# dmosopt/dmosopt

Measured on NVIDIA H100. Metric: candidate-evals/sec (GP+sort+HV) pop=65536 dim=30 obj=3, higher is better.
Workload: dtype f64 results; GP variance contraction in split-fp16 wgmma with fp32 accumulation (precision=auto: calibrated against the float64 path, 0 of 65535 rows of the last step recomputed in float64); ranks on u32 ids

## Files before the change

dmosopt_b200/csrc/common.cuh:

```cuda
#pragma once

#include <cuda_runtime.h>
#include <math.h>
#include <stdint.h>
#include <stdio.h>

#include <string>
#include <vector>

#include "../../include/dmosopt_b200.h"

struct dmo_ctx {
  int device = 0;
  cudaStream_t stream = nullptr;
  cudaMemPool_t pool = nullptr;
  cudaEvent_t ev0 = nullptr, ev1 = nullptr;
  int sm_count = 132;
  int64_t launches = 0;
  int64_t waits = 0;
  std::string err;
  void* flush_buf = nullptr;
  size_t flush_bytes = 0;
  int* dev_flag = nullptr;
  uint64_t h2d_bytes = 0, d2h_bytes = 0;
// ... 216 lines not shown

__device__ __forceinline__ double warp_sum(double v) {
#pragma unroll
  for (int o = 16; o > 0; o >>= 1) v += __shfl_xor_sync(0xffffffffu, v, o);
  return v;
}

template <int NW>
__device__ __forceinline__ double block_sum(double v, double* red) {
  v = warp_sum(v);
  __syncthreads();
  if ((threadIdx.x & 31) == 0) red[threadIdx.x >> 5] = v;
  __syncthreads();
  double s = 0.0;
#pragma unroll 8
  for (int w = 0; w < NW; ++w) s += red[w];
  __syncthreads();
  return s;
}

#endif

int prim_sort_pairs_u64(dmo_ctx* ctx, const uint64_t* kin, uint64_t* kout, const uint32_t* vin,
                        uint32_t* vout, int64_t n, int begin_bit, int end_bit);
int prim_sort_pairs_u32(dmo_ctx* ctx, const uint32_t* kin, uint32_t* kout, const uint32_t* vin,
                        uint32_t* vout, int64_t n, int begin_bit, int end_bit);
int prim_inclusive_sum_u32(dmo_ctx* ctx, const uint32_t* in, uint32_t* out, int64_t n);
int prim_exclusive_sum_i32(dmo_ctx* ctx, const int32_t* in, int32_t* out, int64_t n);
int prim_inclusive_min_f64(dmo_ctx* ctx, const double* in, double* out, int64_t n);
int prim_iota_u32(dmo_ctx* ctx, uint32_t* out, int64_t n);
int prim_gather_u32(dmo_ctx* ctx, const uint32_t* src, const uint32_t* idx, int64_t n, uint32_t* out);
int prim_round_f32(dmo_ctx* ctx, double* a, int64_t n);
int prim_col_keys(dmo_ctx* ctx, const double* dF, int64_t n, int M, int j, uint64_t* keys, uint32_t* idx);
int prim_sort_by_column(dmo_ctx* ctx, const double* dF, int64_t n, int M, int j, DevBuf<uint32_t>& sidx);

int rank_nd_device(dmo_ctx* ctx, const double* dY, int64_t n, int M, int32_t* d_rank);
int rank_nd_device_keep(dmo_ctx* ctx, const double* dY, int64_t n, int M, int64_t keep, int32_t* d_rank);
int nondominated_flags_device(dmo_ctx* ctx, const double* dY, int64_t n, int M, int32_t* d_flag01);
int nondominated_keep_flags(dmo_ctx* ctx, const double* dF, int64_t n, int M, DevBuf<int32_t>& flag);
int dense_ids(dmo_ctx* ctx, const double* dY, int64_t n, int M, DevBuf<uint32_t>& R, DevBuf<uint32_t>& maxid);
int lex_order(dmo_ctx* ctx, const uint32_t* R, int64_t n, int M, int sshift, DevBuf<uint32_t>& permA, DevBuf<uint32_t>& permB,
              const uint32_t** perm);
int crowding_device(dmo_ctx* ctx, const double* dY, int64_t n, int M, double* dD);
int euclidean_device(dmo_ctx* ctx, const double* dY, int64_t n, int M, double* dD);
int lexsort_device(dmo_ctx* ctx, const int32_t* d_rank, const double* const* d_desc_keys, int nkeys,
                   int64_t n, uint32_t* d_perm, bool rank_below_n);
int hypervolume_device(dmo_ctx* ctx, const double* dF, int64_t n, int M, const double* h_ref, double* h_out);
int hypervolume_device_ranked(dmo_ctx* ctx, const double* dF, int64_t n, int M, const double* h_ref, const int32_t* d_rank,
                              double* h_out);
struct Hv3Ranked {
  int64_t n = 0;
  double ref[3] = {0.0, 0.0, 0.0};
  bool tree = false;
  DevBuf<int32_t> pos;
  DevBuf<double> xs, ys, zs, res;
  DevBuf<uint32_t> zo;
};
int hv3_ranked_enqueue(dmo_ctx* ctx, const double* dF, int64_t n, const double* h_ref, const int32_t* d_rank, Hv3Ranked& s);
int hv3_ranked_finish(dmo_ctx* ctx, Hv3Ranked& s, double* h_out);
int tournament_device(dmo_ctx* ctx, const int32_t* d_rank, const double* d_crowd, int64_t pop, int64_t poolsize, uint64_t seed,
                      uint64_t stream_id, int64_t* d_pool, double* d_u);
int nsga2_generate_device(dmo_ctx* ctx, const double* d_pop_x, int d, const int64_t* d_pool, int64_t poolsize, int64_t popsize,
                          double crossover_prob, double mutation_prob, double mutation_rate, const double* d_dic,
                          const double* d_dim, const double* d_xlb, const double* d_xub, uint64_t seed, uint64_t stream_id,
                          double* d_x_gen, int32_t* d_kind, int64_t* n_children, double* d_draws);
int remove_worst_device(dmo_ctx* ctx, const double* dX, const double* dY, int64_t n, int d, int M, int metric,
                        const double* const* d_extra, int n_extra, int64_t keep, double* dX_out, double* dY_out, int32_t* d_rank_out,
                        int64_t* d_perm_out);
int gather_rows_device(dmo_ctx* ctx, const double* src, const double* alt, const uint8_t* sel, const int64_t* idx, int64_t n,
                       int64_t row_elems, double* dst);
int cmaes_generate_device(dmo_ctx* ctx, const double* parents_x, const double* sigmas, int sigma_cols, const double* A,
                          const int64_t* p_idx, const double* z, int64_t n, int d, const double* xlb, const double* xub, double* x_out);
int cmaes_step_z_device(dmo_ctx* ctx, const double* x_gen, const int64_t* cand_idx, const double* parents_x, const int64_t* par_idx,
                        const double* xlb, const double* xub, const double* steps, int64_t n, int d, double* z_out);
int scale_rows_device(dmo_ctx* ctx, double* rows, int64_t row_elems, int64_t n_seg, const int64_t* seg_row, const int64_t* seg_start,
                      const double* factors);
int cmaes_update_cholesky_device(dmo_ctx* ctx, double* A, double* Ainv, double* pc, const double* z, const double* psucc, int64_t n, int d,
                                 double cc, double ccov, double pthresh);
int ehvi_select_device(dmo_ctx* ctx, const double* F, int64_t nf, const double* means, const double* variances, int64_t nc, int M,
                       const double* ref, int nds, int64_t k, int64_t* sel, double* score);
int feas_rank_device(dmo_ctx* ctx, const dmo_feas* m, const double* dX, int64_t n, double* d_rank);
int feas_model_dim(const dmo_feas* m);
```

dmosopt_b200/csrc/gp.cuh:

```cuda
#pragma once
#include <vector>

#include "common.cuh"

struct GpVarOps {
  int64_t Npad = 0;
  int G = 0;
  std::vector<double> h_kscale;
  DevBuf<double> Linv;
  bool tensor_ready = false;
  DevBuf<uint16_t> Lhi, Llo;
  DevBuf<float> Lscale;
  DevBuf<int> Kexp;
  int alloc(dmo_ctx* ctx, int64_t N, int G);
};

struct dmo_gp {
  int64_t N = 0;
  int d = 0, M = 0, kernel = 0;
  bool isotropic = true;
  GpVarOps ops;
  std::vector<int> h_cov, h_lead;
  DevBuf<int> cov;
  DevBuf<double> Xt;
// ... 15 lines not shown
  double cal_mean_err_only = 0.0;
  double cal_var_err = 0.0;
  double refine_theta = 1.0;
  int64_t last_refined = 0;
};

__device__ __forceinline__ double stationary(double s2, int kind) {
  if (kind == DMO_KERNEL_MATERN52) {
    const double K = sqrt(s2) * 2.23606797749978969641;
    return (1.0 + K + K * K / 3.0) * exp(-K);
  }
  return exp(-0.5 * s2);
}

constexpr int64_t GP_MAX_CHUNK = (int64_t)1 << 20;

int gp_predict_fp64(dmo_ctx* ctx, dmo_gp* gp, const double* dXn, int64_t P, double* d_mean, double* d_var);

int gp_linv_from_factor(dmo_ctx* ctx, const double* L, int64_t N, int64_t ldo, double* dst);
int gp_linv_from_factor_batched(dmo_ctx* ctx, const double* L, int64_t ldl, int64_t sL, int64_t N, int nbat, int64_t ldo,
                                int64_t sdst, double* dst);
int gp_fit_batched(dmo_ctx* ctx, int64_t N, int d, int nbat, int kernel, const double* X, const double* inv_ls, const double* constant,
                   const double* diag_add, const double* y, double* A, int64_t ld, int* info, double* work, double* alpha, double* lml);
int gp_potrf_batched(dmo_ctx* ctx, double* A, int64_t ld, int nbat, int* info);
constexpr int GP_F64_TILE = 128;
int gp_var_contract_fp64(dmo_ctx* ctx, const GpVarOps& ops, const double* Ks, int64_t kplane, int64_t Pcpad, int nsplit,
                         double* vnorm, int64_t vn_ld);
int gp_prepare_tensor(dmo_ctx* ctx, GpVarOps& ops);
constexpr int GP_TC_TILE = 128;
int gp_tensor_var_planes(int64_t Npad);
int gp_var_contract_tensor(dmo_ctx* ctx, const GpVarOps& ops, const uint16_t* Kh, const uint16_t* Kl, int64_t k_alloc,
                           int64_t k_rows, int64_t Pcpad, double* vnorm, int64_t vn_ld, int* abort_flag, int free_sms = 0);
#ifndef DMO_GP_LANE_SMS
#define DMO_GP_LANE_SMS 14
#endif
constexpr int GP_LANE_SMS = DMO_GP_LANE_SMS;
struct GpOverlap {
  cudaEvent_t mean_ready = nullptr;
};
int gp_predict_tensor(dmo_ctx* ctx, dmo_gp* gp, const double* dXn, int64_t P, double* d_mean, double* d_var,
                      int* abort_flag = nullptr, const GpOverlap* ov = nullptr, bool var_route_mean = false);
extern const char* const GP_WATCHDOG_MSG;
struct GpPending {
  GpOverlap ov;
  bool active = false;
  int64_t P = 0;
  const double* dXn = nullptr;
  double *d_mean = nullptr, *d_var = nullptr;
  DevBuf<double> xn;
  DevBuf<int32_t> flag, pos;
};
int gp_predict_device(dmo_ctx* ctx, dmo_gp* gp, const double* dX, int64_t P, double* d_mean, double* d_var, int precision,
                      GpPending* pending = nullptr, bool var_route_mean = false);
int gp_predict_finish(dmo_ctx* ctx, dmo_gp* gp, GpPending& pending, bool* refined);

struct GpUnitPredict {
  const char* who = "";
  bool tensor = false;
  int64_t tile = 0;
  int64_t Pc_alloc = 0;
  int n_vp = 0;
  DevBuf<double> vnorm, Ks;
  DevBuf<uint16_t> Kh, Kl;
  DevBuf<int> abort_flag;
  int check(dmo_ctx* ctx, const char* who, int precision, int d);
  int alloc(dmo_ctx* ctx, int64_t P, int64_t Npad, int planes, bool want_var);
  int contract(dmo_ctx* ctx, const GpVarOps& ops, int64_t Pcpad);
// ... 67 lines not shown
```

dmosopt_b200/csrc/hv.cu:

```cuda
#include <stdlib.h>
#include <string.h>

#include "common.cuh"

int hv_many_device(dmo_ctx* ctx, const double* Fnd, const uint32_t* sidx, int64_t n, int M, const double* dref, double* h_out);
int hv3_tree_device(dmo_ctx* ctx, const double* xs, const double* ys, const double* zs, const uint32_t* zo, int64_t n, double rx,
                    double ry, double rz, double* partial, int64_t* n_partial);

namespace {

constexpr int HV_T = 128;

__global__ void inside_flag_kernel(const double* __restrict__ F, int64_t n, int M, const double* __restrict__ ref,
                                   const int32_t* __restrict__ drop, int32_t* __restrict__ flag) {
  int64_t i = (int64_t)blockIdx.x * blockDim.x + threadIdx.x;
  if (i > n) return;
  if (i == n) {
    flag[i] = 0;
    return;
  }
  bool in = drop == nullptr || drop[i] == 0;
  for (int j = 0; j < M; ++j) in = in && (ref[j] > F[i * M + j]);
  flag[i] = in ? 1 : 0;
}
// ... 556 lines not shown
    DMO_TRY(sum_partials(ctx, part_main, n2 * tiles, &t_main));
    DMO_TRY(sum_partials(ctx, part_a, nbv, &t_a));
    if (M == 5) DMO_TRY(sum_partials(ctx, part_b, nbv, &t_b));
    *h_out = (M == 4) ? (t_a - t_main) : (t_a - t_b + t_main);
    return DMO_OK;
  }
  DevBuf<uint32_t> sz, zinv, zo;
  DevBuf<double> xs, ys, zs;
  DMO_TRY(prim_sort_by_column(ctx, Fnd.p, n2, M, 2, sz));
  DMO_TRY(zinv.alloc(ctx, n2));
  DMO_TRY(zo.alloc(ctx, n2));
  DMO_TRY(xs.alloc(ctx, n2));
  DMO_TRY(ys.alloc(ctx, n2));
  DMO_TRY(zs.alloc(ctx, n2));
  const unsigned g = (unsigned)ceil_div(n2, 256);
  DMO_LAUNCH(invert_perm_kernel, g, 256, 0, sz.p, n2, zinv.p);
  DMO_TRY(prim_gather_u32(ctx, zinv.p, sx.p, n2, zo.p));
  DMO_LAUNCH(gather_col_kernel, g, 256, 0, Fnd.p, sx.p, n2, M, 0, xs.p);
  DMO_LAUNCH(gather_col_kernel, g, 256, 0, Fnd.p, sx.p, n2, M, 1, ys.p);
  DMO_LAUNCH(gather_col_kernel, g, 256, 0, Fnd.p, sx.p, n2, M, 2, zs.p);
  int64_t nb = ceil_div(n2, HV_T);
  DevBuf<double> partial;
  DMO_TRY(partial.alloc(ctx, nb));
  if (n2 >= hv3_tree_min()) {
    DMO_TRY(hv3_tree_device(ctx, xs.p, ys.p, zs.p, zo.p, n2, h_ref[0], h_ref[1], h_ref[2], partial.p, &nb));
  } else {
    ProfileScope ps(ctx, "hv3");
    DMO_LAUNCH(hv3_kernel, (unsigned)nb, HV_T, 0, xs.p, ys.p, zs.p, zo.p, n2, h_ref[0], h_ref[1], h_ref[2], partial.p);
  }
  DMO_TRY(sum_partials(ctx, partial, nb, h_out));
  return DMO_OK;
}

int hv3_ranked_enqueue(dmo_ctx* ctx, const double* dF, int64_t n, const double* h_ref, const int32_t* d_rank, Hv3Ranked& s) {
  s.n = n;
  memcpy(s.ref, h_ref, sizeof(s.ref));
  s.tree = n >= hv3_tree_min();
  DevBuf<double> dref, Fin;
  DevBuf<int32_t> flag;
  DevBuf<uint32_t> sx, sz, zinv;
  DMO_TRY(dref.alloc(ctx, 3));
  DMO_CUDA(cudaMemcpyAsync(dref.p, h_ref, 3 * sizeof(double), cudaMemcpyHostToDevice, ctx->stream));
  DMO_TRY(flag.alloc(ctx, n + 1));
  DMO_TRY(s.pos.alloc(ctx, n + 1));
  DMO_TRY(Fin.alloc(ctx, (size_t)n * 3));
  const unsigned g = (unsigned)ceil_div(n, 256);
  DMO_LAUNCH(inside_flag_kernel, (unsigned)ceil_div(n + 1, 256), 256, 0, dF, n, 3, dref.p, d_rank, flag.p);
  DMO_TRY(prim_exclusive_sum_i32(ctx, flag.p, s.pos.p, n + 1));
  DMO_LAUNCH(compact_rows_kernel, g, 256, 0, dF, n, 3, flag.p, s.pos.p, Fin.p);
  DMO_LAUNCH(pad_rows_kernel, g, 256, 0, Fin.p, n, 3, s.pos.p + n, dref.p);
  DMO_TRY(prim_sort_by_column(ctx, Fin.p, n, 3, 0, sx));
  DMO_TRY(prim_sort_by_column(ctx, Fin.p, n, 3, 2, sz));
  DMO_TRY(zinv.alloc(ctx, n));
  DMO_TRY(s.zo.alloc(ctx, n));
  DMO_TRY(s.xs.alloc(ctx, n));
  DMO_TRY(s.ys.alloc(ctx, n));
  DMO_TRY(s.zs.alloc(ctx, n));
  DMO_LAUNCH(invert_perm_kernel, g, 256, 0, sz.p, n, zinv.p);
  DMO_TRY(prim_gather_u32(ctx, zinv.p, sx.p, n, s.zo.p));
  DMO_LAUNCH(gather_col_kernel, g, 256, 0, Fin.p, sx.p, n, 3, 0, s.xs.p);
  DMO_LAUNCH(gather_col_kernel, g, 256, 0, Fin.p, sx.p, n, 3, 1, s.ys.p);
  DMO_LAUNCH(gather_col_kernel, g, 256, 0, Fin.p, sx.p, n, 3, 2, s.zs.p);
  if (s.tree) {
    DevBuf<double> partial;
    int64_t nb = ceil_div(n, HV_T);
    DMO_TRY(partial.alloc(ctx, nb));
    DMO_TRY(hv3_tree_device(ctx, s.xs.p, s.ys.p, s.zs.p, s.zo.p, n, h_ref[0], h_ref[1], h_ref[2], partial.p, &nb));
    DMO_TRY(s.res.alloc(ctx, 1));
    DMO_LAUNCH(final_sum_kernel, 1, 256, 0, partial.p, nb, s.res.p);
  }
  DMO_CHECK_LAUNCH();
  return DMO_OK;
}

int hv3_ranked_finish(dmo_ctx* ctx, Hv3Ranked& s, double* h_out) {
  *h_out = 0.0;
  int32_t n1 = 0;
  DMO_CUDA(cudaMemcpyAsync(&n1, s.pos.p + s.n, sizeof(int32_t), cudaMemcpyDeviceToHost, ctx->stream));
  DMO_CUDA(dmo_wait(ctx));
  if (n1 == 0) return DMO_OK;
  if (s.tree && n1 >= hv3_tree_min()) {
    DMO_CUDA(cudaMemcpyAsync(h_out, s.res.p, sizeof(double), cudaMemcpyDeviceToHost, ctx->stream));
    DMO_CUDA(dmo_wait(ctx));
    return DMO_OK;
  }
// ... 140 lines not shown
```

dmosopt_b200/csrc/prims.cu:

```cuda
#include <cub/cub.cuh>

#include "common.cuh"

int prim_sort_pairs_u64(dmo_ctx* ctx, const uint64_t* kin, uint64_t* kout, const uint32_t* vin,
                        uint32_t* vout, int64_t n, int begin_bit, int end_bit) {
  if (n <= 0) return DMO_OK;
  size_t tmp = 0;
  DMO_CUDA(cub::DeviceRadixSort::SortPairs(nullptr, tmp, kin, kout, vin, vout, (int)n, begin_bit, end_bit,
                                           ctx->stream));
  DevBuf<uint8_t> t;
  DMO_TRY(t.alloc(ctx, tmp));
  DMO_CUDA(cub::DeviceRadixSort::SortPairs(t.p, tmp, kin, kout, vin, vout, (int)n, begin_bit, end_bit,
                                           ctx->stream));
  ctx->launches += 1 + (end_bit - begin_bit + 7) / 8;
  return DMO_OK;
}

int prim_sort_pairs_u32(dmo_ctx* ctx, const uint32_t* kin, uint32_t* kout, const uint32_t* vin,
                        uint32_t* vout, int64_t n, int begin_bit, int end_bit) {
  if (n <= 0) return DMO_OK;
  size_t tmp = 0;
  DMO_CUDA(cub::DeviceRadixSort::SortPairs(nullptr, tmp, kin, kout, vin, vout, (int)n, begin_bit, end_bit,
                                           ctx->stream));
  DevBuf<uint8_t> t;
// ... 62 lines not shown
int prim_gather_u32(dmo_ctx* ctx, const uint32_t* src, const uint32_t* idx, int64_t n, uint32_t* out) {
  if (n <= 0) return DMO_OK;
  DMO_LAUNCH(gather_u32_kernel, (unsigned)ceil_div(n, 256), 256, 0, src, idx, n, out);
  DMO_CHECK_LAUNCH();
  return DMO_OK;
}

__global__ void round_f32_kernel(double* a, int64_t n) {
  int64_t i = (int64_t)blockIdx.x * blockDim.x + threadIdx.x;
  if (i < n) a[i] = (double)(float)a[i];
}

int prim_round_f32(dmo_ctx* ctx, double* a, int64_t n) {
  if (n <= 0) return DMO_OK;
  DMO_LAUNCH(round_f32_kernel, (unsigned)ceil_div(n, 256), 256, 0, a, n);
  DMO_CHECK_LAUNCH();
  return DMO_OK;
}

__global__ void col_key_kernel(const double* __restrict__ F, int64_t n, int M, int j, uint64_t* __restrict__ keys,
                               uint32_t* __restrict__ idx) {
  int64_t i = (int64_t)blockIdx.x * blockDim.x + threadIdx.x;
  if (i < n) {
    keys[i] = f64_to_ordered(F[i * M + j]);
    idx[i] = (uint32_t)i;
  }
}

int prim_col_keys(dmo_ctx* ctx, const double* dF, int64_t n, int M, int j, uint64_t* keys, uint32_t* idx) {
  DMO_LAUNCH(col_key_kernel, (unsigned)ceil_div(n, 256), 256, 0, dF, n, M, j, keys, idx);
  return DMO_OK;
}

int prim_sort_by_column(dmo_ctx* ctx, const double* dF, int64_t n, int M, int j, DevBuf<uint32_t>& sidx) {
  DevBuf<uint64_t> k0, k1;
  DevBuf<uint32_t> i0;
  DMO_TRY(k0.alloc(ctx, n));
  DMO_TRY(k1.alloc(ctx, n));
  DMO_TRY(i0.alloc(ctx, n));
  DMO_TRY(sidx.alloc(ctx, n));
  DMO_TRY(prim_col_keys(ctx, dF, n, M, j, k0.p, i0.p));
  return prim_sort_pairs_u64(ctx, k0.p, k1.p, i0.p, sidx.p, n, 0, 64);
}
```

dmosopt_b200/csrc/rank.cu:

```cuda
#include <stdlib.h>

#include <type_traits>

#include "common.cuh"

namespace {

constexpr int RANK_T = 128;

__device__ __forceinline__ int ld_acquire_gpu(const int* p) {
  int v;
  asm volatile("ld.acquire.gpu.global.s32 %0, [%1];" : "=r"(v) : "l"(p) : "memory");
  return v;
}
__device__ __forceinline__ void st_release_gpu(int* p, int v) {
  asm volatile("st.release.gpu.global.s32 [%0], %1;" ::"l"(p), "r"(v) : "memory");
}

__global__ void flag_new_u64_kernel(const uint64_t* __restrict__ skeys, int64_t n, uint32_t* __restrict__ flag) {
  int64_t p = (int64_t)blockIdx.x * blockDim.x + threadIdx.x;
  if (p < n) flag[p] = (p > 0 && skeys[p] != skeys[p - 1]) ? 1u : 0u;
}

__global__ void scatter_dense_kernel(const uint32_t* __restrict__ dense, const uint32_t* __restrict__ sidx, int64_t n,
// ... 706 lines not shown
  const int j2 = M == 3 ? 2 : 1;
  return GridIds{R, R + n, R + (size_t)j2 * n, maxid + 1, maxid + j2};
}

struct CellGrid {
  int gbits = 0;
  DevBuf<uint32_t> cstartA, cstartB;
  DevBuf<uint4> crecA, crecB;
  DevBuf<uint32_t> pm;
  DevBuf<uint32_t> first, slotA, slotB;
};

__global__ void grid_key_kernel(GridIds ids, int64_t n, int gbits, uint32_t* __restrict__ key0, uint32_t* __restrict__ keyA,
                                uint32_t* __restrict__ keyB) {
  const int64_t i = (int64_t)blockIdx.x * blockDim.x + threadIdx.x;
  if (i >= n) return;
  const uint32_t G1 = (1u << gbits) - 1u;
  const uint32_t a = min(ids.c1[i] >> cell_shift(*ids.max1, gbits), G1), b = min(ids.c2[i] >> cell_shift(*ids.max2, gbits), G1);
  key0[i] = ids.c0[i];
  keyA[i] = (a << gbits) | b;
  keyB[i] = (b << gbits) | a;
}

__global__ void grid_gather_kernel(GridIds ids, const uint32_t* __restrict__ order, int64_t n, uint4* __restrict__ crec,
                                   uint32_t* __restrict__ slot) {
  const int64_t t = (int64_t)blockIdx.x * blockDim.x + threadIdx.x;
  if (t >= n) return;
  const uint32_t i = order[t];
  crec[t] = make_uint4(ids.c0[i], ids.c1[i], ids.c2[i], i);
  if (slot != nullptr) slot[i] = (uint32_t)t;
}

__global__ void grid_start_kernel(const uint32_t* __restrict__ skey, int64_t n, int ncell, uint32_t* __restrict__ cstart) {
  int c = blockIdx.x * blockDim.x + threadIdx.x;
  if (c > ncell) return;
  int64_t lo = 0, hi = n;
  while (lo < hi) {
    const int64_t mid = (lo + hi) >> 1;
    if (skey[mid] < (uint32_t)c) lo = mid + 1; else hi = mid;
  }
  cstart[c] = (uint32_t)lo;
}

__global__ void grid_cellmin_kernel(const uint32_t* __restrict__ cstart, const uint4* __restrict__ crec, int ncell,
                                    uint32_t* __restrict__ first, uint32_t* __restrict__ pm) {
  const int c = blockIdx.x * blockDim.x + threadIdx.x;
  if (c >= ncell) return;
  uint32_t f = first != nullptr ? first[c] : cstart[c];
  const uint32_t e = cstart[c + 1];
  while (f < e && crec[f].x == PEEL_DEAD) ++f;
  if (first != nullptr) first[c] = f;
  pm[c] = f < e ? crec[f].x : PEEL_DEAD;
}

__global__ void grid_prefix_min_kernel(uint32_t* __restrict__ pm, int gbits, int pass) {
  extern __shared__ uint32_t sh_scan[];
  const int G = 1 << gbits;
  const int line = blockIdx.x, t = threadIdx.x;
  const int cell = pass == 0 ? line * G + t : t * G + line;
  uint32_t v = pm[cell];
  sh_scan[t] = v;
  __syncthreads();
  for (int off = 1; off < G; off <<= 1) {
    const uint32_t o = t >= off ? sh_scan[t - off] : PEEL_DEAD;
    __syncthreads();
    v = min(v, o);
    sh_scan[t] = v;
    __syncthreads();
  }
  pm[cell] = v;
}

template <typename OutT>
__global__ void grid_flag_kernel(GridIds ids, int64_t n, int gbits, const uint32_t* __restrict__ pm,
                                 const uint32_t* __restrict__ cstartA, const uint32_t* __restrict__ cstartB,
                                 const uint4* __restrict__ crecA, const uint4* __restrict__ crecB,
                                 const uint8_t* __restrict__ alive, OutT* __restrict__ dom_out) {
  const int64_t i = (int64_t)blockIdx.x * blockDim.x + threadIdx.x;
  if (i >= n || (alive != nullptr && !alive[i])) return;
  const int G = 1 << gbits;
  const uint32_t c0 = ids.c0[i], c1 = ids.c1[i], c2 = ids.c2[i];
  const int a = (int)min(c1 >> cell_shift(*ids.max1, gbits), (uint32_t)(G - 1));
  const int b = (int)min(c2 >> cell_shift(*ids.max2, gbits), (uint32_t)(G - 1));
  bool dom = a > 0 && b > 0 && __ldg(pm + (a - 1) * G + (b - 1)) <= c0;
#pragma unroll
  for (int pass = 0; pass < 2; ++pass) {
    if (dom) break;
    const uint4* cr = pass == 0 ? crecA : crecB;
    uint32_t t = pass == 0 ? __ldg(cstartA + a * G) : __ldg(cstartB + b * G);
    const uint32_t t1 = pass == 0 ? __ldg(cstartA + a * G + b + 1) : __ldg(cstartB + b * G + a);
#define DMO_PEEL_TEST(q) ((q).x <= c0 && (q).y <= c1 && (q).z <= c2 && !((q).x == c0 && (q).y == c1 && (q).z == c2))
    for (; t + 16 <= t1 && !dom; t += 16) {
      uint4 q[16];
#pragma unroll
      for (int u = 0; u < 16; ++u) q[u] = __ldg(cr + t + u);
#pragma unroll
      for (int u = 0; u < 16; ++u) dom = dom || DMO_PEEL_TEST(q[u]);
    }
    for (; t + 4 <= t1 && !dom; t += 4) {
      const uint4 q0 = __ldg(cr + t), q1 = __ldg(cr + t + 1), q2 = __ldg(cr + t + 2), q3 = __ldg(cr + t + 3);
      dom = DMO_PEEL_TEST(q0) || DMO_PEEL_TEST(q1) || DMO_PEEL_TEST(q2) || DMO_PEEL_TEST(q3);
    }
    for (; t < t1 && !dom; ++t) {
      const uint4 q0 = __ldg(cr + t);
      dom = DMO_PEEL_TEST(q0);
    }
#undef DMO_PEEL_TEST
  }
  dom_out[i] = (OutT)(dom ? 1 : 0);
}

int build_cell_grid(dmo_ctx* ctx, const GridIds& ids, int64_t n, int gbits, bool peel, CellGrid& cg) {
  cg.gbits = gbits;
  const int GG = 1 << (2 * gbits);
  const unsigned g = (unsigned)ceil_div(n, 256);
  DevBuf<uint32_t> key0, keyA, keyB, keyS[2], keyT[2], ord0, ordS[2], iota;
  DMO_TRY(key0.alloc(ctx, n));
  DMO_TRY(keyA.alloc(ctx, n));
  DMO_TRY(keyB.alloc(ctx, n));
  for (int pass = 0; pass < 2; ++pass) {
    DMO_TRY(keyS[pass].alloc(ctx, n));
    DMO_TRY(keyT[pass].alloc(ctx, n));
    DMO_TRY(ordS[pass].alloc(ctx, n));
  }
  DMO_TRY(ord0.alloc(ctx, n));
  DMO_TRY(iota.alloc(ctx, n));
  DMO_TRY(cg.cstartA.alloc(ctx, GG + 1));
  DMO_TRY(cg.cstartB.alloc(ctx, GG + 1));
  DMO_TRY(cg.crecA.alloc(ctx, n));
  DMO_TRY(cg.crecB.alloc(ctx, n));
  DMO_TRY(cg.pm.alloc(ctx, GG));
  if (peel) {
    DMO_TRY(cg.first.alloc(ctx, GG));
    DMO_TRY(cg.slotA.alloc(ctx, n));
    DMO_TRY(cg.slotB.alloc(ctx, n));
  }
  DMO_LAUNCH(grid_key_kernel, g, 256, 0, ids, n, gbits, key0.p, keyA.p, keyB.p);
  DMO_TRY(prim_iota_u32(ctx, iota.p, n));
  DMO_TRY(prim_sort_pairs_u32(ctx, key0.p, keyS[0].p, iota.p, ord0.p, n, 0, bits_for(n)));
  {
    SideStreams side(ctx, 2);
    DMO_TRY(side.rc);
    for (int pass = 0; pass < 2; ++pass) {
      side.on(pass);
      DMO_TRY(prim_gather_u32(ctx, pass == 0 ? keyA.p : keyB.p, ord0.p, n, keyT[pass].p));
      DMO_TRY(prim_sort_pairs_u32(ctx, keyT[pass].p, keyS[pass].p, ord0.p, ordS[pass].p, n, 0, 2 * gbits));
      DMO_LAUNCH(grid_gather_kernel, g, 256, 0, ids, ordS[pass].p, n, pass == 0 ? cg.crecA.p : cg.crecB.p,
                 pass == 0 ? cg.slotA.p : cg.slotB.p);
      DMO_LAUNCH(grid_start_kernel, (unsigned)ceil_div(GG + 1, 256), 256, 0, keyS[pass].p, n, GG,
                 pass == 0 ? cg.cstartA.p : cg.cstartB.p);
    }
    side.back();
  }
  if (peel) DMO_CUDA(cudaMemcpyAsync(cg.first.p, cg.cstartA.p, (size_t)GG * sizeof(uint32_t), cudaMemcpyDeviceToDevice, ctx->stream));
  DMO_CHECK_LAUNCH();
  return DMO_OK;
}

template <typename OutT>
int grid_dominated(dmo_ctx* ctx, CellGrid& cg, const GridIds& ids, int64_t n, const uint8_t* alive, OutT* dom) {
  const int G = 1 << cg.gbits, GG = G * G;
  DMO_LAUNCH(grid_cellmin_kernel, (unsigned)ceil_div(GG, 256), 256, 0, cg.cstartA.p, cg.crecA.p, GG, cg.first.p, cg.pm.p);
  DMO_LAUNCH(grid_prefix_min_kernel, G, G, G * sizeof(uint32_t), cg.pm.p, cg.gbits, 0);
  DMO_LAUNCH(grid_prefix_min_kernel, G, G, G * sizeof(uint32_t), cg.pm.p, cg.gbits, 1);
  DMO_LAUNCH((grid_flag_kernel<OutT>), (unsigned)ceil_div(n, 128), 128, 0, ids, n, cg.gbits, cg.pm.p, cg.cstartA.p, cg.cstartB.p,
             cg.crecA.p, cg.crecB.p, alive, dom);
  DMO_CHECK_LAUNCH();
  return DMO_OK;
}

int nd_flags_cell_grid(dmo_ctx* ctx, const uint32_t* R, const uint32_t* maxid, int64_t n, int M, int32_t* d_flag01) {
  int gbits = bits_for(n) / 2;
  if (gbits < 4) gbits = 4;
  if (gbits > 9) gbits = 9;
  const GridIds ids = grid_ids(R, maxid, n, M);
  CellGrid cg;
  ProfileScope ps(ctx, "nd_flags");
  DMO_TRY(build_cell_grid(ctx, ids, n, gbits, false, cg));
  return grid_dominated(ctx, cg, ids, n, nullptr, d_flag01);
}


__global__ void peel_mark_kernel(int64_t n, uint8_t* __restrict__ alive, const uint8_t* __restrict__ dom, int k,
                                 int32_t* __restrict__ rank, const uint32_t* __restrict__ slotA, const uint32_t* __restrict__ slotB,
                                 uint4* __restrict__ crecA, uint4* __restrict__ crecB, unsigned long long* __restrict__ count) {
  const int64_t i = (int64_t)blockIdx.x * blockDim.x + threadIdx.x;
  bool mine = false;
  if (i < n && alive[i] && !dom[i]) {
    mine = true;
    rank[i] = k;
    alive[i] = 0;
    crecA[slotA[i]].x = PEEL_DEAD;
    crecB[slotB[i]].x = PEEL_DEAD;
  }
  const unsigned m = __ballot_sync(0xFFFFFFFFu, mine);
  if ((threadIdx.x & 31) == 0 && m) atomicAdd(count, (unsigned long long)__popc(m));
}

__global__ void peel_rest_kernel(int64_t n, const uint8_t* __restrict__ alive, int k, int32_t* __restrict__ rank) {
  const int64_t i = (int64_t)blockIdx.x * blockDim.x + threadIdx.x;
  if (i < n && alive[i]) rank[i] = k;
}

constexpr int PEEL_PROBE = 256;
__global__ void peel_probe_kernel(const uint32_t* __restrict__ R, int64_t n, unsigned* __restrict__ dominated) {
  __shared__ uint32_t sp[PEEL_PROBE][3];
  __shared__ unsigned sdom[PEEL_PROBE / 32];
  const int64_t stride = n / PEEL_PROBE;
  for (int t = threadIdx.x; t < PEEL_PROBE; t += blockDim.x) {
    const int64_t i = (int64_t)t * stride + (stride >> 1);
    sp[t][0] = R[i];
    sp[t][1] = R[n + i];
    sp[t][2] = R[2 * n + i];
  }
  if (threadIdx.x < PEEL_PROBE / 32) sdom[threadIdx.x] = 0u;
  __syncthreads();
  unsigned mine[PEEL_PROBE / 32];
#pragma unroll
  for (int w = 0; w < PEEL_PROBE / 32; ++w) mine[w] = 0u;
  for (int64_t j = (int64_t)blockIdx.x * blockDim.x + threadIdx.x; j < n; j += (int64_t)gridDim.x * blockDim.x) {
    const uint32_t a = R[j], b = R[n + j], c = R[2 * n + j];
#pragma unroll
    for (int w = 0; w < PEEL_PROBE / 32; ++w) {
      unsigned m = 0u;
#pragma unroll 8
      for (int t = 0; t < 32; ++t) {
        const uint32_t pa = sp[w * 32 + t][0], pb = sp[w * 32 + t][1], pc = sp[w * 32 + t][2];
        const bool d = a <= pa && b <= pb && c <= pc && !(a == pa && b == pb && c == pc);
        m |= d ? (1u << t) : 0u;
      }
      mine[w] |= m;
    }
  }
#pragma unroll
  for (int w = 0; w < PEEL_PROBE / 32; ++w) {
    const unsigned m = __reduce_or_sync(0xFFFFFFFFu, mine[w]);
    if ((threadIdx.x & 31) == 0 && m) atomicOr(&sdom[w], m);
  }
  __syncthreads();
  if (threadIdx.x < PEEL_PROBE / 32 && sdom[threadIdx.x]) atomicOr(&dominated[threadIdx.x], sdom[threadIdx.x]);
}

__global__ void fill_u8_kernel(uint8_t* __restrict__ a, int64_t n, uint8_t v) {
  const int64_t i = (int64_t)blockIdx.x * blockDim.x + threadIdx.x;
  if (i < n) a[i] = v;
}

int rank_by_peeling(dmo_ctx* ctx, const uint32_t* R, const uint32_t* maxid, int64_t n, int64_t keep, int32_t* d_rank, bool* done) {
  *done = false;
  int max_peels = 14;
  if (const char* e = getenv("DMO_RANK_PEEL")) max_peels = atoi(e);
  if (max_peels <= 0) return DMO_OK;
  ProfileScope ps(ctx, "rank_peel");
  double front_guess;
  {
    DevBuf<unsigned> pd;
    DMO_TRY(pd.alloc(ctx, PEEL_PROBE / 32));
    DMO_CUDA(cudaMemsetAsync(pd.p, 0, (PEEL_PROBE / 32) * sizeof(unsigned), ctx->stream));
    const int gridp = (int)(ceil_div(n, 256) < 2 * (int64_t)ctx->sm_count ? ceil_div(n, 256) : 2 * (int64_t)ctx->sm_count);
    DMO_LAUNCH(peel_probe_kernel, gridp, 256, 0, R, n, pd.p);
    DMO_CHECK_LAUNCH();
    unsigned h[PEEL_PROBE / 32];
    DMO_CUDA(cudaMemcpyAsync(h, pd.p, sizeof(h), cudaMemcpyDeviceToHost, ctx->stream));
    DMO_CUDA(dmo_wait(ctx));
    int free_probes = PEEL_PROBE;
    for (int w = 0; w < PEEL_PROBE / 32; ++w) free_probes -= __builtin_popcount(h[w]);
    if (free_probes < 2 && !(getenv("DMO_RANK_PEEL_NOPROBE") && atoi(getenv("DMO_RANK_PEEL_NOPROBE")))) return DMO_OK;
    front_guess = (double)free_probes * (double)n / PEEL_PROBE;
  }
  const int bits = bits_for(n);
  int gbits = (bits + 1) / 2;
  if (gbits < 4) gbits = 4;
  if (const char* e = getenv("DMO_PEEL_GBITS")) gbits = atoi(e);
  if (gbits > 9) gbits = 9;
  const unsigned g = (unsigned)ceil_div(n, 256);
  const GridIds ids = grid_ids(R, maxid, n, 3);
  CellGrid cg;
  DMO_TRY(build_cell_grid(ctx, ids, n, gbits, true, cg));
  DevBuf<uint8_t> alive, dom;
  DevBuf<unsigned long long> count;
  DMO_TRY(alive.alloc(ctx, n));
  DMO_TRY(dom.alloc(ctx, n));
  DMO_TRY(count.alloc(ctx, 1));
  DMO_LAUNCH(fill_u8_kernel, g, 256, 0, alive.p, n, (uint8_t)1);
  DMO_CUDA(cudaMemsetAsync(count.p, 0, sizeof(unsigned long long), ctx->stream));
  DMO_TRY(dmo_lag_slots(ctx));
  auto peel = [&](int j) -> int {
    DMO_TRY(grid_dominated(ctx, cg, ids, n, alive.p, dom.p));
    DMO_LAUNCH(peel_mark_kernel, g, 256, 0, n, alive.p, dom.p, j, d_rank, cg.slotA.p, cg.slotB.p, cg.crecA.p, cg.crecB.p, count.p);
    DMO_CHECK_LAUNCH();
    DMO_CUDA(cudaMemcpyAsync(ctx->lag_host + (j & 1), count.p, sizeof(unsigned long long), cudaMemcpyDeviceToHost, ctx->stream));
    DMO_CUDA(cudaEventRecord(ctx->lag_ev[j & 1], ctx->stream));
    return DMO_OK;
  };
  unsigned long long ranked = 0, before = 0;
  double prev_front = 0.0;
  int k = 0, queued = 1;
  DMO_TRY(peel(0));
  for (;; ++k) {
    if (queued == k + 1 && (double)ranked + front_guess < (double)keep && (k > 0 || front_guess * 64.0 >= (double)keep)) {
      DMO_TRY(peel(k + 1));
      ++queued;
    }
    before = ranked;
    ctx->waits++;
    DMO_CUDA(cudaEventSynchronize(ctx->lag_ev[k & 1]));
    ranked = ctx->lag_host[k & 1];
    if ((int64_t)ranked >= keep || (int64_t)ranked >= n) break;
    const double last = (double)(ranked - before);
    const double grow = last > prev_front ? last - prev_front : 0.0;
    bool give_up;
    if (k == 0) {
      give_up = last * 64.0 < (double)keep;
    } else {
      const double rem = (double)(keep - (int64_t)ranked);
      const double b = last + 0.5 * grow;
      const double ahead = grow > 0.0 ? (-b + sqrt(b * b + 2.0 * grow * rem)) / grow : rem / (last > 0.0 ? last : 1.0);
      give_up = (double)(k + 1) + ahead > (double)max_peels;
    }
    if (give_up) return DMO_OK;
    prev_front = last;
// ... 230 lines not shown
```

dmosopt_b200/csrc/step.cu:

```cuda
#include <string.h>

#include <algorithm>
#include <cmath>

#include "common.cuh"
#include "gp.cuh"

constexpr int kCountWarps = 8;
__global__ void __launch_bounds__(kCountWarps * 32) step_counts_kernel(const int32_t* __restrict__ kind, int64_t P,
                                                                        const int64_t* __restrict__ perm, int64_t pop,
                                                                        unsigned long long* counts) {
  __shared__ double red[kCountWarps];
  double c[4] = {0.0, 0.0, 0.0, 0.0};
  const int64_t n = P > pop ? P : pop;
  for (int64_t i = (int64_t)blockIdx.x * blockDim.x + threadIdx.x; i < n; i += (int64_t)gridDim.x * blockDim.x) {
    if (i < P) {
      const int32_t k = kind[i];
      c[0] += k < 2 ? 1.0 : 0.0;
      c[1] += k == 2 ? 1.0 : 0.0;
    }
    if (i < pop) {
      const int64_t j = perm[i];
      if (j < P) {
        const int32_t k = kind[j];
// ... 131 lines not shown
  if (P > 0) {
    DMO_TRY(rank_in.alloc(ctx, pop));
    DMO_TRY(dmo_lane_streams(ctx));
    gpp.ov.mean_ready = ctx->lane_ev[0];
    ProfileScope ps(ctx, "step_gp");
    DMO_TRY(step_predict(ctx, "nsga2_step", post, Xs.p, P, Ys.p, with_variance ? var.p : nullptr, precision, &gpp));
    if (post.mean_f32) DMO_TRY(prim_round_f32(ctx, Ys.p, P * M));
  }
  auto truncate = [&]() -> int {
    ProfileScope ps(ctx, "step_truncate");
    DMO_TRY(remove_worst_device(ctx, Xs.p, Ys.p, P + pop, d, M, distance_metric, key ? kp : nullptr, key ? 1 : 0, pop, pop_x, pop_y,
                                rank, perm.p));
    if (round_to_f32) DMO_TRY(prim_round_f32(ctx, pop_y, pop * M));
    return DMO_OK;
  };
  auto first_truncate = [&]() -> int {
    if (gpp.active) DMO_CUDA(cudaMemcpyAsync(rank_in.p, rank, (size_t)pop * sizeof(int32_t), cudaMemcpyDeviceToDevice, ctx->stream));
    return truncate();
  };
  auto hypervolume = [&](double* h) -> int {
    ProfileScope ps(ctx, "step_hv");
    return hypervolume_device_ranked(ctx, pop_y, pop, M, h_ref, rank, h);
  };
  Hv3Ranked hv_lane;
  const bool hv_on_lane = want_hv && M == 3 && std::isfinite(h_ref[0]) && std::isfinite(h_ref[1]) && std::isfinite(h_ref[2]);
  bool hv_enqueued = false;
  if (gpp.active && gpp.ov.mean_ready) {
    cudaStream_t main = ctx->stream;
    DMO_CUDA(cudaStreamWaitEvent(ctx->lane, gpp.ov.mean_ready, 0));
    ctx->stream = ctx->lane;
    int rc = first_truncate();
    if (rc == DMO_OK && hv_on_lane) {
      ProfileScope ps(ctx, "step_hv");
      rc = hv3_ranked_enqueue(ctx, pop_y, pop, h_ref, rank, hv_lane);
      hv_enqueued = rc == DMO_OK;
    }
    ctx->stream = main;
    DMO_CUDA(cudaEventRecord(ctx->lane_ev[3], ctx->lane));
    DMO_CUDA(cudaStreamWaitEvent(main, ctx->lane_ev[3], 0));
    DMO_TRY(rc);
  } else {
    DMO_TRY(first_truncate());
  }
  bool refined = false;
  const int rc = gp_predict_finish(ctx, post.gp, gpp, &refined);
  if (rc != DMO_OK) {
    DMO_CUDA(cudaMemcpyAsync(pop_x, Xs.p + (size_t)P * d, (size_t)pop * d * sizeof(double), cudaMemcpyDeviceToDevice, ctx->stream));
    DMO_CUDA(cudaMemcpyAsync(pop_y, Ys.p + (size_t)P * M, (size_t)pop * M * sizeof(double), cudaMemcpyDeviceToDevice, ctx->stream));
    DMO_CUDA(cudaMemcpyAsync(rank, rank_in.p, (size_t)pop * sizeof(int32_t), cudaMemcpyDeviceToDevice, ctx->stream));
    DMO_CUDA(dmo_wait(ctx));
    return rc;
  }
  if (refined) {
    DMO_TRY(truncate());
    hv_enqueued = false;
  }
  if (x_gen) {
    ProfileScope ps(ctx, "step_record");
    DevBuf<unsigned long long> cnt;
    DMO_TRY(cnt.alloc(ctx, 4));
    DMO_CUDA(cudaMemsetAsync(cnt.p, 0, 4 * sizeof(unsigned long long), ctx->stream));
    const int64_t n = P > pop ? P : pop;
    const unsigned grid = (unsigned)std::min<int64_t>(ceil_div(n, kCountWarps * 32), 4 * (int64_t)ctx->sm_count);
    DMO_LAUNCH(step_counts_kernel, grid, kCountWarps * 32, 0, kind.p, P, perm.p, pop, cnt.p);
    DMO_CHECK_LAUNCH();
    DMO_TRY(copy_out(ctx, x_gen, Xs.p, (size_t)P * d * sizeof(double)));
    DMO_TRY(copy_out(ctx, y_gen, Ys.p, (size_t)P * M * sizeof(double)));
// ... 68 lines not shown
```

Before: 9.205 million.

## Rework peel grid scans, reuse grid for probe, and sort HV columns by f32 keys

The cell-start kernel now scatters starts from the sorted keys instead of binary-searching each cell. The column prefix-min becomes a coalesced multi-warp kernel rather than a strided per-line scan. The peel probe reuses the cell grid with one small block instead of a brute-force all-pairs scan. The first peel reuses the precomputed minima. HV3 column sorts use 32-bit float keys when rows are already rounded to f32, and the GP lane SM reservation drops from 14 to 11. Together these aim to cut sort, scan and probe cost in ranking and hypervolume, at the price of relying on f32 rounding being exact for key ordering.

Measured after the change: 9.211 million, median of 6. No clear change (+0.1%).

```diff
diff --git a/dmosopt_b200/csrc/common.cuh b/dmosopt_b200/csrc/common.cuh
--- a/dmosopt_b200/csrc/common.cuh
+++ b/dmosopt_b200/csrc/common.cuh
@@ -272,7 +272,7 @@
 int prim_gather_u32(dmo_ctx* ctx, const uint32_t* src, const uint32_t* idx, int64_t n, uint32_t* out);
 int prim_round_f32(dmo_ctx* ctx, double* a, int64_t n);
 int prim_col_keys(dmo_ctx* ctx, const double* dF, int64_t n, int M, int j, uint64_t* keys, uint32_t* idx);
-int prim_sort_by_column(dmo_ctx* ctx, const double* dF, int64_t n, int M, int j, DevBuf<uint32_t>& sidx);
+int prim_sort_by_column(dmo_ctx* ctx, const double* dF, int64_t n, int M, int j, DevBuf<uint32_t>& sidx, bool f32_keys = false);
 
 int rank_nd_device(dmo_ctx* ctx, const double* dY, int64_t n, int M, int32_t* d_rank);
 int rank_nd_device_keep(dmo_ctx* ctx, const double* dY, int64_t n, int M, int64_t keep, int32_t* d_rank);
@@ -296,7 +296,8 @@
   DevBuf<double> xs, ys, zs, res;
   DevBuf<uint32_t> zo;
 };
-int hv3_ranked_enqueue(dmo_ctx* ctx, const double* dF, int64_t n, const double* h_ref, const int32_t* d_rank, Hv3Ranked& s);
+int hv3_ranked_enqueue(dmo_ctx* ctx, const double* dF, int64_t n, const double* h_ref, const int32_t* d_rank, bool f32_rows,
+                       Hv3Ranked& s);
 int hv3_ranked_finish(dmo_ctx* ctx, Hv3Ranked& s, double* h_out);
 int tournament_device(dmo_ctx* ctx, const int32_t* d_rank, const double* d_crowd, int64_t pop, int64_t poolsize, uint64_t seed,
                       uint64_t stream_id, int64_t* d_pool, double* d_u);
diff --git a/dmosopt_b200/csrc/gp.cuh b/dmosopt_b200/csrc/gp.cuh
--- a/dmosopt_b200/csrc/gp.cuh
+++ b/dmosopt_b200/csrc/gp.cuh
@@ -71,7 +71,7 @@
 int gp_var_contract_tensor(dmo_ctx* ctx, const GpVarOps& ops, const uint16_t* Kh, const uint16_t* Kl, int64_t k_alloc,
                            int64_t k_rows, int64_t Pcpad, double* vnorm, int64_t vn_ld, int* abort_flag, int free_sms = 0);
 #ifndef DMO_GP_LANE_SMS
-#define DMO_GP_LANE_SMS 14
+#define DMO_GP_LANE_SMS 11
 #endif
 constexpr int GP_LANE_SMS = DMO_GP_LANE_SMS;
 struct GpOverlap {
diff --git a/dmosopt_b200/csrc/hv.cu b/dmosopt_b200/csrc/hv.cu
--- a/dmosopt_b200/csrc/hv.cu
+++ b/dmosopt_b200/csrc/hv.cu
@@ -612,7 +612,8 @@
   return DMO_OK;
 }
 
-int hv3_ranked_enqueue(dmo_ctx* ctx, const double* dF, int64_t n, const double* h_ref, const int32_t* d_rank, Hv3Ranked& s) {
+int hv3_ranked_enqueue(dmo_ctx* ctx, const double* dF, int64_t n, const double* h_ref, const int32_t* d_rank, bool f32_rows,
+                       Hv3Ranked& s) {
   s.n = n;
   memcpy(s.ref, h_ref, sizeof(s.ref));
   s.tree = n >= hv3_tree_min();
@@ -629,8 +630,8 @@
   DMO_TRY(prim_exclusive_sum_i32(ctx, flag.p, s.pos.p, n + 1));
   DMO_LAUNCH(compact_rows_kernel, g, 256, 0, dF, n, 3, flag.p, s.pos.p, Fin.p);
   DMO_LAUNCH(pad_rows_kernel, g, 256, 0, Fin.p, n, 3, s.pos.p + n, dref.p);
-  DMO_TRY(prim_sort_by_column(ctx, Fin.p, n, 3, 0, sx));
-  DMO_TRY(prim_sort_by_column(ctx, Fin.p, n, 3, 2, sz));
+  DMO_TRY(prim_sort_by_column(ctx, Fin.p, n, 3, 0, sx, f32_rows));
+  DMO_TRY(prim_sort_by_column(ctx, Fin.p, n, 3, 2, sz, f32_rows));
   DMO_TRY(zinv.alloc(ctx, n));
   DMO_TRY(s.zo.alloc(ctx, n));
   DMO_TRY(s.xs.alloc(ctx, n));
diff --git a/dmosopt_b200/csrc/prims.cu b/dmosopt_b200/csrc/prims.cu
--- a/dmosopt_b200/csrc/prims.cu
+++ b/dmosopt_b200/csrc/prims.cu
@@ -118,13 +118,29 @@
   return DMO_OK;
 }
 
-int prim_sort_by_column(dmo_ctx* ctx, const double* dF, int64_t n, int M, int j, DevBuf<uint32_t>& sidx) {
+__global__ void col_key_f32_kernel(const double* __restrict__ F, int64_t n, int M, int j, uint32_t* __restrict__ keys,
+                                   uint32_t* __restrict__ idx) {
+  int64_t i = (int64_t)blockIdx.x * blockDim.x + threadIdx.x;
+  if (i < n) {
+    keys[i] = f32_to_ordered(__double2float_ru(F[i * M + j]));
+    idx[i] = (uint32_t)i;
+  }
+}
+
+int prim_sort_by_column(dmo_ctx* ctx, const double* dF, int64_t n, int M, int j, DevBuf<uint32_t>& sidx, bool f32_keys) {
+  DMO_TRY(sidx.alloc(ctx, n));
+  DevBuf<uint32_t> i0;
+  DMO_TRY(i0.alloc(ctx, n));
+  if (f32_keys) {
+    DevBuf<uint32_t> k0, k1;
+    DMO_TRY(k0.alloc(ctx, n));
+    DMO_TRY(k1.alloc(ctx, n));
+    DMO_LAUNCH(col_key_f32_kernel, (unsigned)ceil_div(n, 256), 256, 0, dF, n, M, j, k0.p, i0.p);
+    return prim_sort_pairs_u32(ctx, k0.p, k1.p, i0.p, sidx.p, n, 0, 32);
+  }
   DevBuf<uint64_t> k0, k1;
-  DevBuf<uint32_t> i0;
   DMO_TRY(k0.alloc(ctx, n));
   DMO_TRY(k1.alloc(ctx, n));
-  DMO_TRY(i0.alloc(ctx, n));
-  DMO_TRY(sidx.alloc(ctx, n));
   DMO_TRY(prim_col_keys(ctx, dF, n, M, j, k0.p, i0.p));
   return prim_sort_pairs_u64(ctx, k0.p, k1.p, i0.p, sidx.p, n, 0, 64);
 }
diff --git a/dmosopt_b200/csrc/rank.cu b/dmosopt_b200/csrc/rank.cu
--- a/dmosopt_b200/csrc/rank.cu
+++ b/dmosopt_b200/csrc/rank.cu
@@ -762,14 +762,11 @@
 }
 
 __global__ void grid_start_kernel(const uint32_t* __restrict__ skey, int64_t n, int ncell, uint32_t* __restrict__ cstart) {
-  int c = blockIdx.x * blockDim.x + threadIdx.x;
-  if (c > ncell) return;
-  int64_t lo = 0, hi = n;
-  while (lo < hi) {
-    const int64_t mid = (lo + hi) >> 1;
-    if (skey[mid] < (uint32_t)c) lo = mid + 1; else hi = mid;
-  }
-  cstart[c] = (uint32_t)lo;
+  const int64_t t = (int64_t)blockIdx.x * blockDim.x + threadIdx.x;
+  if (t > n) return;
+  const int64_t lo = t == 0 ? 0 : (int64_t)skey[t - 1] + 1;
+  const int64_t hi = t == n ? ncell : min((int64_t)skey[t], (int64_t)ncell);
+  for (int64_t c = lo; c <= hi; ++c) cstart[c] = (uint32_t)t;
 }
 
 __global__ void grid_cellmin_kernel(const uint32_t* __restrict__ cstart, const uint4* __restrict__ crec, int ncell,
@@ -783,11 +780,11 @@
   pm[c] = f < e ? crec[f].x : PEEL_DEAD;
 }
 
-__global__ void grid_prefix_min_kernel(uint32_t* __restrict__ pm, int gbits, int pass) {
+__global__ void grid_row_min_kernel(uint32_t* __restrict__ pm, int gbits) {
   extern __shared__ uint32_t sh_scan[];
   const int G = 1 << gbits;
-  const int line = blockIdx.x, t = threadIdx.x;
-  const int cell = pass == 0 ? line * G + t : t * G + line;
+  const int t = threadIdx.x;
+  const int cell = blockIdx.x * G + t;
   uint32_t v = pm[cell];
   sh_scan[t] = v;
   __syncthreads();
@@ -801,13 +798,36 @@
   pm[cell] = v;
 }
 
-template <typename OutT>
-__global__ void grid_flag_kernel(GridIds ids, int64_t n, int gbits, const uint32_t* __restrict__ pm,
-                                 const uint32_t* __restrict__ cstartA, const uint32_t* __restrict__ cstartB,
-                                 const uint4* __restrict__ crecA, const uint4* __restrict__ crecB,
-                                 const uint8_t* __restrict__ alive, OutT* __restrict__ dom_out) {
-  const int64_t i = (int64_t)blockIdx.x * blockDim.x + threadIdx.x;
-  if (i >= n || (alive != nullptr && !alive[i])) return;
+constexpr int GRID_COL_WARPS = 16;
+__global__ void __launch_bounds__(GRID_COL_WARPS * 32) grid_col_min_kernel(uint32_t* __restrict__ pm, int gbits) {
+  __shared__ uint32_t tot[GRID_COL_WARPS][32];
+  const int G = 1 << gbits, rows = G / GRID_COL_WARPS;
+  const int cx = threadIdx.x & 31, wg = threadIdx.x >> 5;
+  const int c = blockIdx.x * 32 + cx;
+  const bool on = c < G;
+  uint32_t v[512 / GRID_COL_WARPS];
+#pragma unroll
+  for (int k = 0; k < 512 / GRID_COL_WARPS; ++k)
+    if (on && k < rows) v[k] = pm[(size_t)(wg * rows + k) * G + c];
+  uint32_t run = PEEL_DEAD;
+#pragma unroll
+  for (int k = 0; k < 512 / GRID_COL_WARPS; ++k)
+    if (on && k < rows) {
+      run = min(run, v[k]);
+      v[k] = run;
+    }
+  tot[wg][cx] = run;
+  __syncthreads();
+  uint32_t above = PEEL_DEAD;
+  for (int w = 0; w < wg; ++w) above = min(above, tot[w][cx]);
+#pragma unroll
+  for (int k = 0; k < 512 / GRID_COL_WARPS; ++k)
+    if (on && k < rows) pm[(size_t)(wg * rows + k) * G + c] = min(above, v[k]);
+}
+
+__device__ __forceinline__ bool grid_dominates(const GridIds& ids, int64_t i, int gbits, const uint32_t* __restrict__ pm,
+                                               const uint32_t* __restrict__ cstartA, const uint32_t* __restrict__ cstartB,
+                                               const uint4* __restrict__ crecA, const uint4* __restrict__ crecB) {
   const int G = 1 << gbits;
   const uint32_t c0 = ids.c0[i], c1 = ids.c1[i], c2 = ids.c2[i];
   const int a = (int)min(c1 >> cell_shift(*ids.max1, gbits), (uint32_t)(G - 1));
@@ -837,7 +857,17 @@
     }
 #undef DMO_PEEL_TEST
   }
-  dom_out[i] = (OutT)(dom ? 1 : 0);
+  return dom;
+}
+
+template <typename OutT>
+__global__ void grid_flag_kernel(GridIds ids, int64_t n, int gbits, const uint32_t* __restrict__ pm,
+                                 const uint32_t* __restrict__ cstartA, const uint32_t* __restrict__ cstartB,
+                                 const uint4* __restrict__ crecA, const uint4* __restrict__ crecB,
+                                 const uint8_t* __restrict__ alive, OutT* __restrict__ dom_out) {
+  const int64_t i = (int64_t)blockIdx.x * blockDim.x + threadIdx.x;
+  if (i >= n || (alive != nullptr && !alive[i])) return;
+  dom_out[i] = (OutT)(grid_dominates(ids, i, gbits, pm, cstartA, cstartB, crecA, crecB) ? 1 : 0);
 }
 
 int build_cell_grid(dmo_ctx* ctx, const GridIds& ids, int64_t n, int gbits, bool peel, CellGrid& cg) {
@@ -877,7 +907,7 @@
       DMO_TRY(prim_sort_pairs_u32(ctx, keyT[pass].p, keyS[pass].p, ord0.p, ordS[pass].p, n, 0, 2 * gbits));
       DMO_LAUNCH(grid_gather_kernel, g, 256, 0, ids, ordS[pass].p, n, pass == 0 ? cg.crecA.p : cg.crecB.p,
                  pass == 0 ? cg.slotA.p : cg.slotB.p);
-      DMO_LAUNCH(grid_start_kernel, (unsigned)ceil_div(GG + 1, 256), 256, 0, keyS[pass].p, n, GG,
+      DMO_LAUNCH(grid_start_kernel, (unsigned)ceil_div(n + 1, 256), 256, 0, keyS[pass].p, n, GG,
                  pass == 0 ? cg.cstartA.p : cg.cstartB.p);
     }
     side.back();
@@ -887,14 +917,27 @@
   return DMO_OK;
 }
 
+int grid_minima(dmo_ctx* ctx, CellGrid& cg) {
+  const int G = 1 << cg.gbits, GG = G * G;
+  DMO_LAUNCH(grid_cellmin_kernel, (unsigned)ceil_div(GG, 256), 256, 0, cg.cstartA.p, cg.crecA.p, GG, cg.first.p, cg.pm.p);
+  DMO_LAUNCH(grid_row_min_kernel, G, G, G * sizeof(uint32_t), cg.pm.p, cg.gbits);
+  DMO_LAUNCH(grid_col_min_kernel, (unsigned)ceil_div(G, 32), GRID_COL_WARPS * 32, 0, cg.pm.p, cg.gbits);
+  DMO_CHECK_LAUNCH();
+  return DMO_OK;
+}
+
+template <typename OutT>
+int grid_flags(dmo_ctx* ctx, CellGrid& cg, const GridIds& ids, int64_t n, const uint8_t* alive, OutT* dom) {
+  DMO_LAUNCH((grid_flag_kernel<OutT>), (unsigned)ceil_div(n, 128), 128, 0, ids, n, cg.gbits, cg.pm.p, cg.cstartA.p, cg.cstartB.p,
+             cg.crecA.p, cg.crecB.p, alive, dom);
+  DMO_CHECK_LAUNCH();
+  return DMO_OK;
+}
+
 template <typename OutT>
 int grid_dominated(dmo_ctx* ctx, CellGrid& cg, const GridIds& ids, int64_t n, const uint8_t* alive, OutT* dom) {
-  const int G = 1 << cg.gbits, GG = G * G;
-  DMO_LAUNCH(grid_cellmin_kernel, (unsigned)ceil_div(GG, 256), 256, 0, cg.cstartA.p, cg.crecA.p, GG, cg.first.p, cg.pm.p);
-  DMO_LAUNCH(grid_prefix_min_kernel, G, G, G * sizeof(uint32_t), cg.pm.p, cg.gbits, 0);
-  DMO_LAUNCH(grid_prefix_min_kernel, G, G, G * sizeof(uint32_t), cg.pm.p, cg.gbits, 1);
-  DMO_LAUNCH((grid_flag_kernel<OutT>), (unsigned)ceil_div(n, 128), 128, 0, ids, n, cg.gbits, cg.pm.p, cg.cstartA.p, cg.cstartB.p,
-             cg.crecA.p, cg.crecB.p, alive, dom);
+  DMO_TRY(grid_minima(ctx, cg));
+  return grid_flags(ctx, cg, ids, n, alive, dom);
   DMO_CHECK_LAUNCH();
   return DMO_OK;
 }
@@ -933,42 +976,14 @@
 }
 
 constexpr int PEEL_PROBE = 256;
-__global__ void peel_probe_kernel(const uint32_t* __restrict__ R, int64_t n, unsigned* __restrict__ dominated) {
-  __shared__ uint32_t sp[PEEL_PROBE][3];
-  __shared__ unsigned sdom[PEEL_PROBE / 32];
+__global__ void __launch_bounds__(PEEL_PROBE) peel_probe_kernel(GridIds ids, int64_t n, int gbits, const uint32_t* __restrict__ pm,
+                                                                const uint32_t* __restrict__ cstartA, const uint32_t* __restrict__ cstartB,
+                                                                const uint4* __restrict__ crecA, const uint4* __restrict__ crecB,
+                                                                unsigned* __restrict__ dominated) {
   const int64_t stride = n / PEEL_PROBE;
-  for (int t = threadIdx.x; t < PEEL_PROBE; t += blockDim.x) {
-    const int64_t i = (int64_t)t * stride + (stride >> 1);
-    sp[t][0] = R[i];
-    sp[t][1] = R[n + i];
-    sp[t][2] = R[2 * n + i];
-  }
-  if (threadIdx.x < PEEL_PROBE / 32) sdom[threadIdx.x] = 0u;
-  __syncthreads();
-  unsigned mine[PEEL_PROBE / 32];
-#pragma unroll
-  for (int w = 0; w < PEEL_PROBE / 32; ++w) mine[w] = 0u;
-  for (int64_t j = (int64_t)blockIdx.x * blockDim.x + threadIdx.x; j < n; j += (int64_t)gridDim.x * blockDim.x) {
-    const uint32_t a = R[j], b = R[n + j], c = R[2 * n + j];
-#pragma unroll
-    for (int w = 0; w < PEEL_PROBE / 32; ++w) {
-      unsigned m = 0u;
-#pragma unroll 8
-      for (int t = 0; t < 32; ++t) {
-        const uint32_t pa = sp[w * 32 + t][0], pb = sp[w * 32 + t][1], pc = sp[w * 32 + t][2];
-        const bool d = a <= pa && b <= pb && c <= pc && !(a == pa && b == pb && c == pc);
-        m |= d ? (1u << t) : 0u;
-      }
-      mine[w] |= m;
-    }
-  }
-#pragma unroll
-  for (int w = 0; w < PEEL_PROBE / 32; ++w) {
-    const unsigned m = __reduce_or_sync(0xFFFFFFFFu, mine[w]);
-    if ((threadIdx.x & 31) == 0 && m) atomicOr(&sdom[w], m);
-  }
-  __syncthreads();
-  if (threadIdx.x < PEEL_PROBE / 32 && sdom[threadIdx.x]) atomicOr(&dominated[threadIdx.x], sdom[threadIdx.x]);
+  const int64_t i = (int64_t)threadIdx.x * stride + (stride >> 1);
+  const unsigned m = __ballot_sync(0xFFFFFFFFu, grid_dominates(ids, i, gbits, pm, cstartA, cstartB, crecA, crecB));
+  if ((threadIdx.x & 31) == 0) dominated[threadIdx.x >> 5] = m;
 }
 
 __global__ void fill_u8_kernel(uint8_t* __restrict__ a, int64_t n, uint8_t v) {
@@ -982,13 +997,21 @@
   if (const char* e = getenv("DMO_RANK_PEEL")) max_peels = atoi(e);
   if (max_peels <= 0) return DMO_OK;
   ProfileScope ps(ctx, "rank_peel");
+  const int bits = bits_for(n);
+  int gbits = (bits + 1) / 2;
+  if (const char* e = getenv("DMO_PEEL_GBITS")) gbits = atoi(e);
+  if (gbits < 4) gbits = 4;
+  if (gbits > 9) gbits = 9;
+  const unsigned g = (unsigned)ceil_div(n, 256);
+  const GridIds ids = grid_ids(R, maxid, n, 3);
+  CellGrid cg;
+  DMO_TRY(build_cell_grid(ctx, ids, n, gbits, true, cg));
+  DMO_TRY(grid_minima(ctx, cg));
   double front_guess;
   {
     DevBuf<unsigned> pd;
     DMO_TRY(pd.alloc(ctx, PEEL_PROBE / 32));
-    DMO_CUDA(cudaMemsetAsync(pd.p, 0, (PEEL_PROBE / 32) * sizeof(unsigned), ctx->stream));
-    const int gridp = (int)(ceil_div(n, 256) < 2 * (int64_t)ctx->sm_count ? ceil_div(n, 256) : 2 * (int64_t)ctx->sm_count);
-    DMO_LAUNCH(peel_probe_kernel, gridp, 256, 0, R, n, pd.p);
+    DMO_LAUNCH(peel_probe_kernel, 1, PEEL_PROBE, 0, ids, n, gbits, cg.pm.p, cg.cstartA.p, cg.cstartB.p, cg.crecA.p, cg.crecB.p, pd.p);
     DMO_CHECK_LAUNCH();
     unsigned h[PEEL_PROBE / 32];
     DMO_CUDA(cudaMemcpyAsync(h, pd.p, sizeof(h), cudaMemcpyDeviceToHost, ctx->stream));
@@ -998,15 +1021,6 @@
     if (free_probes < 2 && !(getenv("DMO_RANK_PEEL_NOPROBE") && atoi(getenv("DMO_RANK_PEEL_NOPROBE")))) return DMO_OK;
     front_guess = (double)free_probes * (double)n / PEEL_PROBE;
   }
-  const int bits = bits_for(n);
-  int gbits = (bits + 1) / 2;
-  if (gbits < 4) gbits = 4;
-  if (const char* e = getenv("DMO_PEEL_GBITS")) gbits = atoi(e);
-  if (gbits > 9) gbits = 9;
-  const unsigned g = (unsigned)ceil_div(n, 256);
-  const GridIds ids = grid_ids(R, maxid, n, 3);
-  CellGrid cg;
-  DMO_TRY(build_cell_grid(ctx, ids, n, gbits, true, cg));
   DevBuf<uint8_t> alive, dom;
   DevBuf<unsigned long long> count;
   DMO_TRY(alive.alloc(ctx, n));
@@ -1016,7 +1030,8 @@
   DMO_CUDA(cudaMemsetAsync(count.p, 0, sizeof(unsigned long long), ctx->stream));
   DMO_TRY(dmo_lag_slots(ctx));
   auto peel = [&](int j) -> int {
-    DMO_TRY(grid_dominated(ctx, cg, ids, n, alive.p, dom.p));
+    if (j > 0) DMO_TRY(grid_minima(ctx, cg));
+    DMO_TRY(grid_flags(ctx, cg, ids, n, alive.p, dom.p));
     DMO_LAUNCH(peel_mark_kernel, g, 256, 0, n, alive.p, dom.p, j, d_rank, cg.slotA.p, cg.slotB.p, cg.crecA.p, cg.crecB.p, count.p);
     DMO_CHECK_LAUNCH();
     DMO_CUDA(cudaMemcpyAsync(ctx->lag_host + (j & 1), count.p, sizeof(unsigned long long), cudaMemcpyDeviceToHost, ctx->stream));
diff --git a/dmosopt_b200/csrc/step.cu b/dmosopt_b200/csrc/step.cu
--- a/dmosopt_b200/csrc/step.cu
+++ b/dmosopt_b200/csrc/step.cu
@@ -187,7 +187,7 @@
     int rc = first_truncate();
     if (rc == DMO_OK && hv_on_lane) {
       ProfileScope ps(ctx, "step_hv");
-      rc = hv3_ranked_enqueue(ctx, pop_y, pop, h_ref, rank, hv_lane);
+      rc = hv3_ranked_enqueue(ctx, pop_y, pop, h_ref, rank, round_to_f32 != 0, hv_lane);
       hv_enqueued = rc == DMO_OK;
     }
     ctx->stream = main;
```
